# tusen-ai/SST

Hardware: AMD Instinct MI355X
Metric: LiDAR frames/sec (SST backbone fwd+bwd) at Waymo 0.32m voxels (higher is better)
Workload: dtype f32 (storage, accumulation, attention, LayerNorm, reductions: fp32; the dense products of the encoder layers from the EXACT three-way bf16 split of both fp32 operands, six bf16 MFMA products with fp32 accumulation - error vs float64 <= 2 x the fp32 matrix pipe's: tests/test_gpu_dense_f32x6.py)

## Files before the change

### include/sst_amd.h

```cpp
#ifndef SST_AMD_H
#define SST_AMD_H

#include <stdint.h>

#ifdef __cplusplus
extern "C" {
#endif

#define SST_OK 0
#define SST_ERR_ARG (-1)
#define SST_ERR_UNSUPPORTED (-2)
#define SST_ERR_KEYSPACE (-3)

typedef enum { SST_REDUCE_SUM = 0, SST_REDUCE_MEAN = 1, SST_REDUCE_MAX = 2 } sst_reduce_t;

const char* sst_version(void);

int sst_dynamic_voxelize_f32(const float* d_points, int64_t n, int64_t row_stride,
                             const float voxel_size[3], const float coors_range[6],
                             int32_t* d_coors, int64_t coors_stride, int coors_col0, int batch_idx,
                             void* stream);
void sst_dynamic_voxelize_grid(const float voxel_size[3], const float coors_range[6], int32_t grid_xyz[3]);

int64_t sst_scan_workspace_bytes(int64_t n);
// ... 184 lines not shown
int sst_add_layernorm_act_bwd_f32(const float* d_dy, const float* d_sum, const float* d_stats, const float* d_weight,
                                  const float* d_bias, int act, int64_t m, int c, float* d_dx, float* d_dweight,
                                  float* d_dbias, void* d_workspace, void* stream);
int sst_add_layernorm_fwd_f32(const float* d_x, const float* d_res, const float* d_weight, const float* d_bias,
                              int64_t m, int c, float eps, float* d_y, float* d_sum, float* d_stats,
                              void* stream);
int sst_add_layernorm_pos_fwd_f32(const float* d_x, const float* d_res, const float* d_weight, const float* d_bias, int64_t m,
                                  int c, float eps, float* d_y, float* d_sum, float* d_stats, const float* d_pos_table,
                                  const int32_t* d_pos_idx, float* d_y_plus_pos, void* stream);
int64_t sst_add_layernorm_bwd_workspace_bytes(int64_t m, int c);
int sst_add_layernorm_bwd_f32(const float* d_dy, const float* d_sum, const float* d_stats,
                              const float* d_weight, int64_t m, int c, float* d_dx, float* d_dweight,
                              float* d_dbias, void* d_workspace, void* stream);
int64_t sst_colsum_workspace_bytes(int64_t m, int c);
int sst_colsum_f32(const float* d_x, int64_t m, int c, int64_t ld, float* d_out, void* d_workspace, void* stream);

int64_t sst_weight_grad_workspace_bytes(int64_t m, int out, int in);
int sst_weight_grad_f32(const float* d_dy, const float* d_x, int64_t m, int out, int in, int64_t ld_dy,
                        int64_t ld_x, float* d_dw, float* d_db, void* d_workspace, void* stream);
typedef struct sst_wgrad_problem_f32 {
  const float* dy;
  const float* x;
  int64_t m, ld_dy, ld_x;
  float* dw;
  float* db;
  int32_t out, in;
  const float* x_add_rows;
  const int32_t* x_add_index;
} sst_wgrad_problem_f32;
int64_t sst_weight_grad_group_workspace_bytes(const sst_wgrad_problem_f32* problems, int n);
int sst_weight_grad_group_f32(const sst_wgrad_problem_f32* problems, int n, void* d_workspace, void* stream);
int64_t sst_weight_grad_group_f32x6_workspace_bytes(const sst_wgrad_problem_f32* problems, int n);
int sst_weight_grad_group_f32x6(const sst_wgrad_problem_f32* problems, int n, void* d_workspace, void* stream);

int64_t sst_bn_workspace_bytes(int64_t n, int c);
int sst_bn_stats_f32(const float* d_x, int64_t n, int c, int64_t ld, float* d_mean, float* d_var,
                     void* d_workspace, void* stream);
int sst_bn_act_fwd_f32(const float* d_x, int64_t n, int c, int64_t ldx, const float* d_scale,
                       const float* d_shift, int act, float* d_y, int64_t ldy, void* stream);
int sst_bn_act_bwd_reduce_f32(const float* d_dy, const float* d_x, int64_t n, int c, int64_t lddy, int64_t ldx,
                              const float* d_mean, const float* d_invstd, const float* d_scale,
                              const float* d_shift, int act, float* d_sum_g, float* d_sum_gxhat,
                              void* d_workspace, void* stream);
int sst_bn_act_bwd_apply_f32(const float* d_dy, const float* d_x, int64_t n, int c, int64_t lddy, int64_t ldx,
                             const float* d_mean, const float* d_invstd, const float* d_scale,
                             const float* d_shift, const float* d_coef_a, const float* d_coef_b, float coef_scale,
                             int act, float* d_dx, int64_t lddx, void* stream);
int sst_bn_prepare_f32(const float* d_x, int64_t n, int c, int64_t ld, const float* d_weight, const float* d_bias,
                       float eps, float* d_running_mean, float* d_running_var, float factor, float* d_out4,
                       void* d_workspace, void* stream);
int sst_bn_prepare_tracked_f32(const float* d_x, int64_t n, int c, int64_t ld, const float* d_weight,
                               const float* d_bias, float eps, float* d_running_mean, float* d_running_var,
                               float factor, int64_t* d_num_batches_tracked, float* d_out4, void* d_workspace,
                               void* stream);
int sst_vfe_linear_moments_f32(const float* d_x, int64_t ldx, int64_t n, int k, const float* d_w, int64_t ldw, int c,
                               float* d_y, int64_t ldy, void* d_workspace, void* stream);
int sst_bn_prepare_from_partials_f32(int64_t n, int c, const float* d_weight, const float* d_bias, float eps,
                                     float* d_running_mean, float* d_running_var, float factor,
                                     int64_t* d_num_batches_tracked, float* d_out4, void* d_workspace, void* stream);
int sst_bn_stats_from_partials_f32(int64_t n, int c, float* d_mean, float* d_var, void* d_workspace, void* stream);
int sst_bn_act_pool_bwd_reduce_f32(const float* d_dy, const float* d_x, int64_t n, int c, int64_t lddy, int64_t ldx,
                                   const float* d_mean, const float* d_invstd, const float* d_scale, const float* d_shift,
                                   int act, const int32_t* d_group, const int32_t* d_arg, const float* d_dpool, int64_t ldp,
                                   float* d_sum_g, float* d_sum_gxhat, void* d_workspace, void* stream);
int sst_bn_act_pool_bwd_apply_f32(const float* d_dy, const float* d_x, int64_t n, int c, int64_t lddy, int64_t ldx,
                                  const float* d_mean, const float* d_invstd, const float* d_scale, const float* d_shift,
// ... 352 lines not shown
```

### sst_amd/_lib.py

```python
import ctypes
import os
import subprocess

import torch

_HERE = os.path.dirname(os.path.abspath(__file__))
_CSRC = os.path.join(_HERE, 'csrc')
LIB_PATH = os.path.join(_CSRC, 'libsst_amd.so')

_lib = None

c_i64 = ctypes.c_int64
c_i32 = ctypes.c_int
c_f32 = ctypes.c_float
c_ptr = ctypes.c_void_p



class WgradProblemBF16(ctypes.Structure):
    _fields_ = [('a', c_ptr), ('b', c_ptr), ('lda', c_i64), ('ldb', c_i64), ('m', c_i64), ('out_w', c_ptr),
                ('out_b', c_ptr), ('p', ctypes.c_int32), ('bias_side', ctypes.c_int32),
                ('transpose_out', ctypes.c_int32), ('reserved', ctypes.c_int32)]


# ... 137 lines not shown
    'sst_sra_attn_fwd_ord_f32': (c_i32, [c_ptr, c_ptr, c_ptr, c_i64, c_i64, c_i64, c_ptr, c_ptr, c_ptr, c_i64, c_i32,
                                         c_f32, c_i32, c_i32, c_ptr, c_i64, c_ptr, c_ptr]),
    'sst_sra_attn_bwd_ord_f32': (c_i32, [c_ptr] * 6 + [c_i64] * 5 + [c_ptr, c_ptr, c_ptr, c_i64, c_i64, c_i32, c_f32,
                                                                     c_i32, c_i32, c_ptr, c_ptr, c_ptr,
                                                                     c_i64, c_i64, c_i64, c_ptr, c_ptr]),
    'sst_sra_attn_bwd_workspace_bytes': (c_i64, [c_i64, c_i32]),
    'sst_sra_attn_cos_fwd_f32': (c_i32, [c_ptr, c_ptr, c_ptr, c_i64, c_i64, c_i64, c_ptr, c_ptr, c_ptr, c_i64, c_i32,
                                         c_ptr, c_i32, c_ptr, c_i64, c_ptr, c_ptr]),
    'sst_sra_attn_cos_bwd_f32': (c_i32, [c_ptr] * 6 + [c_i64] * 5 + [c_ptr, c_ptr, c_ptr, c_i64, c_i64, c_i32, c_ptr,
                                                                     c_i32, c_ptr, c_ptr, c_ptr,
                                                                     c_i64, c_i64, c_i64, c_ptr, c_ptr]),
    'sst_sra_attn_fwd_bf16': (c_i32, [c_ptr, c_ptr, c_ptr, c_i64, c_i64, c_i64, c_ptr, c_ptr, c_i64, c_i32, c_f32, c_i32,
                                      c_ptr, c_i64, c_ptr, c_ptr]),
    'sst_sra_attn_bwd_bf16': (c_i32, [c_ptr] * 6 + [c_i64] * 5 + [c_ptr, c_ptr, c_i64, c_i32, c_f32, c_i32, c_ptr, c_ptr,
                                                                  c_ptr, c_i64, c_i64, c_i64, c_ptr]),
    'sst_sra_attn_bf16_profile_next': (c_i32, [c_i32, c_ptr, c_ptr]),
    'sst_sra_attn_fwd_ord_bf16': (c_i32, [c_ptr, c_ptr, c_ptr, c_i64, c_i64, c_i64, c_ptr, c_ptr, c_ptr, c_i64, c_i32, c_f32,
                                          c_i32, c_ptr, c_i64, c_ptr, c_ptr]),
    'sst_sra_attn_bwd_ord_bf16': (c_i32, [c_ptr] * 6 + [c_i64] * 5 + [c_ptr, c_ptr, c_ptr, c_i64, c_i32, c_f32, c_i32, c_ptr,
                                                                      c_ptr, c_ptr, c_i64, c_i64, c_i64, c_ptr]),
    'sst_sra_attn_cos_fwd_bf16': (c_i32, [c_ptr, c_ptr, c_ptr, c_i64, c_i64, c_i64, c_ptr, c_ptr, c_ptr, c_i64, c_i32, c_ptr,
                                          c_i32, c_ptr, c_i64, c_ptr, c_ptr]),
    'sst_sra_attn_cos_bwd_bf16': (c_i32, [c_ptr] * 6 + [c_i64] * 5 + [c_ptr, c_ptr, c_ptr, c_i64, c_i32, c_ptr, c_i32, c_ptr,
                                                                      c_ptr, c_ptr, c_i64, c_i64, c_i64, c_ptr, c_ptr]),
    'sst_add_layernorm_fwd_bf16': (c_i32, [c_ptr, c_ptr, c_ptr, c_ptr, c_i64, c_i32, c_f32, c_ptr, c_ptr, c_ptr, c_ptr,
                                           c_ptr, c_ptr, c_ptr]),
    'sst_add_layernorm_bwd_bf16': (c_i32, [c_ptr, c_ptr, c_ptr, c_ptr, c_ptr, c_i64, c_i32, c_ptr, c_ptr, c_ptr, c_ptr,
                                           c_ptr]),
    'sst_cast_add_pos_bf16': (c_i32, [c_ptr, c_i32, c_i64, c_i32, c_ptr, c_ptr, c_ptr, c_ptr]),
    'sst_weight_grad_group_workspace_bytes': (c_i64, [c_ptr, c_i32]),
    'sst_weight_grad_group_f32': (c_i32, [c_ptr, c_i32, c_ptr, c_ptr]),
    'sst_weight_grad_group_f32x6_workspace_bytes': (c_i64, [c_ptr, c_i32]),
    'sst_weight_grad_group_f32x6': (c_i32, [c_ptr, c_i32, c_ptr, c_ptr]),
    'sst_tall_linear_ln_f32': (c_i32, [c_ptr, c_i64, c_ptr, c_i64, c_ptr, c_i64, c_i32, c_ptr, c_i64, c_ptr, c_ptr, c_f32, c_ptr,
                                       c_ptr, c_ptr, c_ptr, c_ptr, c_ptr, c_ptr]),
    'sst_tall_linear_ln_f32x3': (c_i32, [c_ptr, c_i64, c_ptr, c_i64, c_ptr, c_i64, c_i32, c_ptr, c_i64, c_ptr, c_ptr, c_f32, c_ptr,
                                         c_ptr, c_ptr, c_ptr, c_ptr, c_ptr, c_ptr]),
    'sst_tall_linear_epi_f32x3': (c_i32, [c_ptr, c_i64, c_ptr, c_i64, c_i32, c_ptr, c_i64, c_i32, c_i32, c_i32, c_ptr, c_ptr,
                                          c_i64, c_ptr, c_i64, c_ptr]),
    'sst_tall_linear_ln_f32x6': (c_i32, [c_ptr, c_i64, c_ptr, c_i64, c_ptr, c_i64, c_i32, c_ptr, c_i64, c_ptr, c_ptr, c_f32, c_ptr,
                                         c_ptr, c_ptr, c_ptr, c_ptr, c_ptr, c_ptr]),
    'sst_tall_linear_epi_f32x6': (c_i32, [c_ptr, c_i64, c_ptr, c_i64, c_i32, c_ptr, c_i64, c_i32, c_i32, c_i32, c_ptr, c_ptr,
                                          c_i64, c_ptr, c_i64, c_ptr]),
    'sst_tall_linear_epi2_f32x6': (c_i32, [c_ptr, c_ptr, c_i32, c_i64, c_ptr, c_i64, c_i32, c_ptr, c_i64, c_i32, c_i32, c_i32,
                                           c_ptr, c_ptr, c_i64, c_ptr, c_i64, c_ptr]),
    'sst_add_layernorm_bwd2_f32': (c_i32, [c_ptr, c_ptr, c_ptr, c_ptr, c_ptr, c_i64, c_i32, c_ptr, c_ptr, c_ptr, c_ptr, c_ptr]),
    'sst_tall_linear_epi_f32': (c_i32, [c_ptr, c_i64, c_ptr, c_i64, c_i32, c_ptr, c_i64, c_i32, c_i32, c_i32, c_ptr, c_ptr,
                                        c_i64, c_ptr, c_i64, c_ptr]),
    'sst_tall_linear_bf16': (c_i32, [c_ptr, c_i64, c_ptr, c_ptr, c_i64, c_i32, c_i32, c_i32, c_ptr, c_ptr, c_i64, c_ptr,
                                     c_i64, c_ptr]),
    'sst_tall_linear_ln_bf16': (c_i32, [c_ptr, c_i64, c_ptr, c_ptr, c_i64, c_i32, c_ptr, c_i64, c_ptr, c_ptr, c_f32, c_ptr, c_ptr,
                                        c_ptr, c_ptr, c_ptr, c_ptr, c_ptr]),
    'sst_wgrad_group_workspace_bytes': (c_i64, [c_ptr, c_i32]),
    'sst_wgrad_group_bf16': (c_i32, [c_ptr, c_i32, c_ptr, c_ptr]),
    'sst_cast_group_bf16': (c_i32, [c_ptr, c_i32, c_ptr]),
    'sst_gather_rows_f32': (c_i32, [c_ptr, c_i64, c_ptr, c_i64, c_i32, c_f32, c_ptr, c_i64, c_ptr]),
    'sst_add_table_rows_f32': (c_i32, [c_ptr, c_i64, c_ptr, c_i64, c_ptr, c_i64, c_i32, c_ptr, c_i64, c_ptr]),
    'sst_scatter_rows_f32': (c_i32, [c_ptr, c_i64, c_ptr, c_i64, c_i32, c_ptr, c_i64, c_ptr]),
    'sst_add_layernorm_fwd_f32': (c_i32, [c_ptr, c_ptr, c_ptr, c_ptr, c_i64, c_i32, c_f32, c_ptr, c_ptr, c_ptr,
                                          c_ptr]),
    'sst_add_layernorm_bwd_workspace_bytes': (c_i64, [c_i64, c_i32]),
    'sst_add_layernorm_pos_fwd_f32': (c_i32, [c_ptr, c_ptr, c_ptr, c_ptr, c_i64, c_i32, c_f32, c_ptr, c_ptr, c_ptr, c_ptr, c_ptr,
                                              c_ptr, c_ptr]),
    'sst_add_layernorm_act_fwd_f32': (c_i32, [c_ptr, c_ptr, c_ptr, c_ptr, c_i64, c_i32, c_f32, c_i32, c_ptr, c_ptr, c_ptr,
                                              c_ptr]),
    'sst_add_layernorm_act_bwd_f32': (c_i32, [c_ptr, c_ptr, c_ptr, c_ptr, c_ptr, c_i32, c_i64, c_i32, c_ptr, c_ptr, c_ptr,
# ... 241 lines not shown
```

### sst_amd/csrc/wgrad_x6.hip

```cpp
#include <math.h>
#include <stdlib.h>
#include "common.h"

namespace {

typedef float f32x4 __attribute__((ext_vector_type(4)));
typedef float f32x2 __attribute__((ext_vector_type(2)));
typedef unsigned u32x4 __attribute__((ext_vector_type(4)));
typedef unsigned u32x2 __attribute__((ext_vector_type(2)));
typedef __bf16 bf16x8 __attribute__((ext_vector_type(8)));
typedef __bf16 bf16x2 __attribute__((ext_vector_type(2)));

__device__ __forceinline__ unsigned pack2(float lo, float hi) {
  const f32x2 v = {lo, hi};
  return __builtin_bit_cast(unsigned, __builtin_convertvector(v, bf16x2));
}
__device__ __forceinline__ float lo_f(unsigned p) { return __uint_as_float(p << 16); }
__device__ __forceinline__ float hi_f(unsigned p) { return __uint_as_float(p & 0xffff0000u); }
__device__ __forceinline__ f32x4 mma32(u32x4 a, u32x4 b, f32x4 c) {
  return __builtin_amdgcn_mfma_f32_16x16x32_bf16(__builtin_bit_cast(bf16x8, a), __builtin_bit_cast(bf16x8, b), c, 0, 0, 0);
}
__device__ __forceinline__ void split2(float a, float b, unsigned& p0, unsigned& p1, unsigned& p2) {
  p0 = pack2(a, b);
  const float ra = a - lo_f(p0), rb = b - hi_f(p0);
  p1 = pack2(ra, rb);
  p2 = pack2(ra - lo_f(p1), rb - hi_f(p1));
}

constexpr int kMaxProblems = 8;
constexpr int kTile = 128;
constexpr int kStep = 32;
constexpr int kTileLds = 1040;
constexpr int kImage = 8 * kTileLds;
constexpr int kStage = 2 * 3 * kImage;
constexpr int kLdsBytes = 2 * kStage;

struct x6_problem {
  const float* dy;
  const float* x;
  int64_t m, ld_dy, ld_x;
  int out, in;
  int tile0;
  int db_off;
  float* dw;
  float* db;
  const float* x_add_rows;
  const int32_t* x_add_index;
};
struct x6_group {
  x6_problem p[kMaxProblems];
  int n, tiles, slices;
  int64_t tokens_per_slice;
};

__global__ __launch_bounds__(512, 2) void wgrad_x6_k(const x6_group G, float* __restrict__ part, float* __restrict__ dbp) {
  extern __shared__ __attribute__((aligned(16))) unsigned char lds[];
  const int tid = threadIdx.x, lane = tid & 63, wave = tid >> 6;
  const int l15 = lane & 15, g = lane >> 4;
  const int tile = blockIdx.x / G.slices, slice = blockIdx.x - tile * G.slices;
  int pi = 0;
#pragma unroll
  for (int q = 1; q < kMaxProblems; ++q)
    if (q < G.n && tile >= G.p[q].tile0) pi = q;
  const x6_problem P = G.p[pi];
  const int tiles_k = P.in / kTile;
  const int tl = tile - P.tile0, tn = tl / tiles_k, tk = tl - tn * tiles_k;
  const int n0 = tn * kTile, k0 = tk * kTile;
  const int64_t t_begin = (int64_t)slice * G.tokens_per_slice;
  int64_t t_end = t_begin + G.tokens_per_slice;
  t_end = t_end < P.m ? t_end : P.m;

  const int op = tid >> 8, tq = (tid >> 5) & 7, cg = tid & 31;
  const float* src = op == 0 ? P.dy + n0 + 4 * cg : P.x + k0 + 4 * cg;
  const int64_t ld = op == 0 ? P.ld_dy : P.ld_x;
  const int st_off = (cg >> 2) * kTileLds + (tq & 1) * 512 + (tq >> 1) * 128 + (cg & 3) * 32;
  constexpr int kPf = 2;
  f32x4 rows[kPf][4];
  const int64_t t_last = t_end > 0 ? t_end - 1 : 0;
  const bool xadd = op == 1 && P.x_add_rows != nullptr;
  const float* addsrc = xadd ? P.x_add_rows + k0 + 4 * cg : nullptr;
  f32x4 prow[kPf][4];
  int32_t pidx[4] = {0, 0, 0, 0};
  auto load_idx = [&](int64_t t0) {
#pragma unroll
    for (int r = 0; r < 4; ++r) {
      int64_t t = t0 + 4 * tq + r;
      t = t < t_last ? t : t_last;
      pidx[r] = P.x_add_index[t];
    }
  };
  auto load_rows = [&](int64_t t0, f32x4 (&dst)[4], f32x4 (&pdst)[4]) {
#pragma unroll
    for (int r = 0; r < 4; ++r) {
      int64_t t = t0 + 4 * tq + r;
      t = t < t_last ? t : t_last;
      dst[r] = *(const f32x4*)(src + t * ld);
    }
    if (xadd) {
#pragma unroll
      for (int r = 0; r < 4; ++r) pdst[r] = *(const f32x4*)(addsrc + (int64_t)pidx[r] * P.in);
      load_idx(t0 + kStep);
    }
  };
  float bsum[4] = {0.f, 0.f, 0.f, 0.f};
  u32x4 img[3][2];
  auto split_col = [&](int e, int64_t t0, const f32x4 (&rws)[4], const f32x4 (&prw)[4]) {
    float v[4];
#pragma unroll
    for (int r = 0; r < 4; ++r) v[r] = (t0 + 4 * tq + r < t_end) ? (xadd ? rws[r][e] + prw[r][e] : rws[r][e]) : 0.f;
    if (op == 0) bsum[e] += (v[0] + v[1]) + (v[2] + v[3]);
    unsigned a0, a1, a2, b0, b1, b2;
    split2(v[0], v[1], a0, a1, a2);
    split2(v[2], v[3], b0, b1, b2);
    img[0][e >> 1][2 * (e & 1)] = a0;
    img[0][e >> 1][2 * (e & 1) + 1] = b0;
    img[1][e >> 1][2 * (e & 1)] = a1;
    img[1][e >> 1][2 * (e & 1) + 1] = b1;
    img[2][e >> 1][2 * (e & 1)] = a2;
    img[2][e >> 1][2 * (e & 1) + 1] = b2;
  };
  auto store_img = [&](int buf) {
    unsigned char* base = lds + buf * kStage + op * 3 * kImage + st_off;
#pragma unroll
    for (int im = 0; im < 3; ++im) {
      *(u32x4*)(base + im * kImage) = img[im][0];
      *(u32x4*)(base + im * kImage + 16) = img[im][1];
    }
  };
  const int wn = wave & 3, wk = wave >> 2;
  const int frag_off = g * 128 + l15 * 8;
  f32x4 acc[4][2], acl[4][2];
#pragma unroll
  for (int a = 0; a < 4; ++a)
#pragma unroll
    for (int b = 0; b < 2; ++b) acc[a][b] = acl[a][b] = (f32x4){0.f, 0.f, 0.f, 0.f};
  auto frag = [&](const unsigned char* image, int tile16) -> u32x4 {
    const unsigned char* p = image + tile16 * kTileLds + frag_off;
    const u32x2 lo = *(const u32x2*)p, hi = *(const u32x2*)(p + 512);
    return (u32x4){lo[0], lo[1], hi[0], hi[1]};
  };

  if (xadd) load_idx(t_begin);
#pragma unroll
  for (int u = 0; u < kPf; ++u) load_rows(t_begin + (int64_t)u * kStep, rows[u], prow[u]);
#pragma unroll
  for (int e = 0; e < 4; ++e) split_col(e, t_begin, rows[0], prow[0]);
  store_img(0);
  load_rows(t_begin + (int64_t)kPf * kStep, rows[0], prow[0]);
  __syncthreads();
  const int64_t n_steps = (t_end - t_begin + kStep - 1) / kStep;
  for (int64_t s0 = 0; s0 < n_steps; s0 += kPf) {
#pragma unroll
    for (int u = 0; u < kPf; ++u) {
      const int64_t s = s0 + u;
      if (s >= n_steps) break;
      const int64_t t1 = t_begin + (s + 1) * kStep;
      const unsigned char* dyi = lds + (u & 1) * kStage;
      const unsigned char* xi = dyi + 3 * kImage;
      u32x4 b0[2], b1[2], b2[2];
#pragma unroll
      for (int b = 0; b < 2; ++b) {
        b0[b] = frag(dyi, 2 * wn + b);
        b1[b] = frag(dyi + kImage, 2 * wn + b);
        b2[b] = frag(dyi + 2 * kImage, 2 * wn + b);
      }
#pragma unroll
      for (int a = 0; a < 4; ++a) {
        const u32x4 a0 = frag(xi, 4 * wk + a), a1 = frag(xi + kImage, 4 * wk + a), a2 = frag(xi + 2 * kImage, 4 * wk + a);
#pragma unroll
        for (int b = 0; b < 2; ++b) acl[a][b] = mma32(a2, b0[b], acl[a][b]);
#pragma unroll
        for (int b = 0; b < 2; ++b) acl[a][b] = mma32(a0, b2[b], acl[a][b]);
#pragma unroll
        for (int b = 0; b < 2; ++b) acl[a][b] = mma32(a1, b1[b], acl[a][b]);
#pragma unroll
        for (int b = 0; b < 2; ++b) acl[a][b] = mma32(a1, b0[b], acl[a][b]);
#pragma unroll
        for (int b = 0; b < 2; ++b) acl[a][b] = mma32(a0, b1[b], acl[a][b]);
#pragma unroll
        for (int b = 0; b < 2; ++b) acc[a][b] = mma32(a0, b0[b], acc[a][b]);
        split_col(a, t1, rows[(u + 1) % kPf], prow[(u + 1) % kPf]);
      }
      store_img((u + 1) & 1);
      load_rows(t1 + (int64_t)kPf * kStep, rows[(u + 1) % kPf], prow[(u + 1) % kPf]);
      __syncthreads();
    }
  }
#pragma unroll
  for (int a = 0; a < 4; ++a)
#pragma unroll
    for (int b = 0; b < 2; ++b) acc[a][b] += acl[a][b];
  float* dst = part + ((int64_t)tile * G.slices + slice) * (kTile * kTile);
#pragma unroll
  for (int a = 0; a < 4; ++a)
#pragma unroll
    for (int b = 0; b < 2; ++b)
      *(f32x4*)(dst + (32 * wn + 16 * b + l15) * kTile + 64 * wk + 16 * a + 4 * g) = acc[a][b];
  if (P.db_off >= 0 && tk == 0) {
    float* red = (float*)lds;
    if (op == 0) *(f32x4*)(red + tq * 128 + 4 * cg) = (f32x4){bsum[0], bsum[1], bsum[2], bsum[3]};
    __syncthreads();
    if (tid < 128) {
      float s = 0.f;
#pragma unroll
      for (int q = 0; q < 8; ++q) s += red[q * 128 + tid];
      dbp[((int64_t)P.db_off + n0 + tid) * G.slices + slice] = s;
    }
  }
}

struct x6_riders {
  sst_colsum_rider r[2];
  int n, blocks0;
};

constexpr int kRedQuads = 32, kRedGroups = 8;

__global__ __launch_bounds__(256) void wgrad_x6_reduce_k(const x6_group G, const float* __restrict__ part,
                                                         const float* __restrict__ dbp, int rider_blocks,
                                                         const x6_riders R) {
  __shared__ double red[kRedGroups][kRedQuads][4];
  if ((int)blockIdx.x < rider_blocks) {
    const int second = (int)blockIdx.x >= R.blocks0 ? 1 : 0;
    const sst_colsum_rider& J = R.r[second];
    const int rblk = (int)blockIdx.x - (second ? R.blocks0 : 0);
    float* fr = (float*)&red[0][0][0];
    const int cx = threadIdx.x & 31, gq = threadIdx.x >> 5;
    const int i = rblk * 32 + cx;
    float acc[4] = {0.f, 0.f, 0.f, 0.f};
    if (i < J.width) {
      const float* src = J.partials + i;
      for (int base = 0; base < J.nb; base += 512) {
        float v[16][4];
#pragma unroll
        for (int it = 0; it < 16; ++it)
#pragma unroll
          for (int j = 0; j < 4; ++j) {
            const int b = base + 32 * it + gq + 8 * j;
            v[it][j] = src[(int64_t)(b < J.nb ? b : J.nb - 1) * J.width];
          }
#pragma unroll
        for (int it = 0; it < 16; ++it)
#pragma unroll
          for (int j = 0; j < 4; ++j)
            if (base + 32 * it + gq + 8 * j < J.nb) acc[j] += v[it][j];
      }
    }
#pragma unroll
    for (int j = 0; j < 4; ++j) fr[(gq + 8 * j) * 33 + cx] = acc[j];
    __syncthreads();
    if (gq == 0 && i < J.width) {
      float t = 0.f;
#pragma unroll
      for (int k = 0; k < 32; ++k) t += fr[k * 33 + cx];
      if (i < J.split)
        J.out0[i] = t;
      else
        J.out1[i - J.split] = t;
    }
    return;
  }
  const int blk = (int)blockIdx.x - rider_blocks;
  const int ql = threadIdx.x & (kRedQuads - 1), sg = threadIdx.x / kRedQuads;
  const int64_t quad = (int64_t)blk * kRedQuads + ql;
  const int64_t tile = quad / (kTile * kTile / 4);
  const int e4 = (int)(quad - tile * (kTile * kTile / 4));
  double d0 = 0.0, d1 = 0.0, d2 = 0.0, d3 = 0.0;
  if (tile < G.tiles) {
    const float* src = part + tile * G.slices * (int64_t)(kTile * kTile) + 4 * e4;
#pragma unroll 8
    for (int q = sg; q < G.slices; q += kRedGroups) {
      const f32x4 v = *(const f32x4*)(src + (int64_t)q * (kTile * kTile));
      d0 += v[0], d1 += v[1], d2 += v[2], d3 += v[3];
    }
  }
  red[sg][ql][0] = d0, red[sg][ql][1] = d1, red[sg][ql][2] = d2, red[sg][ql][3] = d3;
  __syncthreads();
  if (sg == 0 && tile < G.tiles) {
    f32x4 s;
#pragma unroll
    for (int r = 0; r < 4; ++r) {
      double t = 0.0;
#pragma unroll
      for (int k = 0; k < kRedGroups; ++k) t += red[k][ql][r];
      s[r] = (float)t;
    }
    int pi = 0;
#pragma unroll
    for (int q = 1; q < kMaxProblems; ++q)
      if (q < G.n && tile >= G.p[q].tile0) pi = q;
    const int tiles_k = G.p[pi].in / kTile;
    const int tl = (int)tile - G.p[pi].tile0, tn = tl / tiles_k, tk = tl - tn * tiles_k;
    const int n = tn * kTile + e4 / 32, k = tk * kTile + (e4 % 32) * 4;
    *(f32x4*)(G.p[pi].dw + (int64_t)n * G.p[pi].in + k) = s;
  }
  const int64_t col = (int64_t)blk * 256 + threadIdx.x;
  int base = 0;
  for (int q = 0; q < G.n; ++q) {
    if (G.p[q].db_off < 0) continue;
    if (col >= base && col < base + G.p[q].out) {
      const float* src = dbp + ((int64_t)G.p[q].db_off + (col - base)) * G.slices;
      double s = 0.0;
      for (int i = 0; i < G.slices; ++i) s += src[i];
      G.p[q].db[col - base] = (float)s;
    }
    base += G.p[q].out;
  }
}

bool aligned16(const void* p) { return ((uintptr_t)p & 15) == 0; }

struct x6_plan {
  x6_group g;
  int64_t part_bytes, db_bytes;
};

bool make_plan(const sst_wgrad_problem_f32* pr, int n, x6_plan* plan) {
  if (!pr || n < 1 || n > kMaxProblems) return false;
  x6_group& G = plan->g;
  G.n = n;
  int tiles = 0, db_cols = 0;
  int64_t m = pr[0].m;
  for (int i = 0; i < n; ++i) {
    const sst_wgrad_problem_f32& p = pr[i];
    if (p.m != m || p.m < 1 || p.out < kTile || p.in < kTile || (p.out % kTile) || (p.in % kTile) || (p.ld_dy & 3) ||
        (p.ld_x & 3) || !p.dy || !p.x || !p.dw || !aligned16(p.dy) || !aligned16(p.x) || !aligned16(p.dw))
      return false;
    G.p[i].dy = p.dy;
    G.p[i].x = p.x;
    G.p[i].m = p.m;
    G.p[i].ld_dy = p.ld_dy;
    G.p[i].ld_x = p.ld_x;
    G.p[i].out = p.out;
    G.p[i].in = p.in;
    G.p[i].tile0 = tiles;
    G.p[i].db_off = p.db ? db_cols : -1;
    G.p[i].dw = p.dw;
    G.p[i].db = p.db;
    if ((p.x_add_rows != nullptr) != (p.x_add_index != nullptr) || (p.x_add_rows && !aligned16(p.x_add_rows))) return false;
    G.p[i].x_add_rows = p.x_add_rows;
    G.p[i].x_add_index = p.x_add_index;
    tiles += (p.out / kTile) * (p.in / kTile);
    if (p.db) db_cols += p.out;
  }
  G.tiles = tiles;
  int slices = (256 / tiles) & ~7;
  if (slices < 8) slices = 8;
  const int64_t max_slices = sst_div_up(m, (int64_t)kStep);
  while (slices > 8 && slices > max_slices) slices -= 8;
  G.slices = slices;
  G.tokens_per_slice = sst_align_up(sst_div_up(m, (int64_t)slices), (int64_t)kStep);
  plan->part_bytes = sst_align_up((int64_t)tiles * slices * kTile * kTile * 4, 256);
  plan->db_bytes = sst_align_up((int64_t)(db_cols > 0 ? db_cols : 1) * slices * 4, 256);
  return true;
}

}

extern "C" {

int64_t sst_weight_grad_group_f32x6_workspace_bytes(const sst_wgrad_problem_f32* problems, int n) {
  x6_plan plan;
  if (!make_plan(problems, n, &plan)) return SST_ERR_UNSUPPORTED;
  return plan.part_bytes + plan.db_bytes;
}

}

int sst_internal_weight_grad_group_f32x6(const sst_wgrad_problem_f32* problems, int n, void* d_workspace,
                                         const sst_colsum_rider* riders, int n_riders, void* stream) {
  x6_plan plan;
  if (!make_plan(problems, n, &plan)) return SST_ERR_UNSUPPORTED;
  if (!d_workspace || !aligned16(d_workspace)) return SST_ERR_ARG;
  hipStream_t st = (hipStream_t)stream;
  float* part = (float*)d_workspace;
  float* dbp = (float*)((char*)d_workspace + plan.part_bytes);
  static unsigned long long configured = 0;
  if (sst_first_use_on_device(&configured)) {
    SST_HIP(hipFuncSetAttribute((const void*)wgrad_x6_k, hipFuncAttributeMaxDynamicSharedMemorySize, kLdsBytes));
    sst_mark_device(&configured);
  }
  const int64_t quads = (int64_t)plan.g.tiles * (kTile * kTile / 4);
  const int tile_blocks = (int)sst_div_up(quads, (int64_t)kRedQuads);
  if (n_riders < 0 || n_riders > 2 || (n_riders > 0 && !riders)) return SST_ERR_ARG;
  x6_riders R;
  R.n = n_riders, R.blocks0 = 0;
  int extra = 0;
  for (int i = 0; i < n_riders; ++i) {
    const sst_colsum_rider& q = riders[i];
    if (!q.partials || q.nb < 1 || q.width < 1 || !q.out0 || !q.out1) return SST_ERR_ARG;
    R.r[i] = q;
    if (i == 0) R.blocks0 = (q.width + 31) / 32;
    extra += (q.width + 31) / 32;
  }
  hipLaunchKernelGGL(wgrad_x6_k, dim3((unsigned)(plan.g.tiles * plan.g.slices)), dim3(512), kLdsBytes, st, plan.g, part, dbp);
  hipLaunchKernelGGL(wgrad_x6_reduce_k, dim3((unsigned)(tile_blocks + extra)), dim3(256), 0, st, plan.g, part, dbp, extra, R);
  SST_LAUNCH_CHECK();
  return SST_OK;
}

extern "C" {

int sst_weight_grad_group_f32x6(const sst_wgrad_problem_f32* problems, int n, void* d_workspace, void* stream) {
  return sst_internal_weight_grad_group_f32x6(problems, n, d_workspace, nullptr, 0, stream);
}

}
```

Measured before the change: 97.91.

## Pair adjacent weight-grad tiles per block to reuse the shared operand split

The f32x6 weight-gradient kernel now processes units of two adjacent 128x128 output tiles along the in or out dimension. Each unit loads and splits the shared operand (dy or x) once and reuses it for both tiles. It uses 256-thread blocks with a three-block LDS stage and larger per-wave accumulators. Leftover odd tiles run as single-tile units. The host planner picks separate slice counts for pairs and singles from a cost model over 256 CUs. The reduce kernel and bias reduction are updated for the new partial layout, and a partition query API is added. This cuts redundant global loads and bf16 splitting, at the cost of more register pressure, occupancy 1, and fewer blocks per tile.

```diff
diff --git a/include/sst_amd.h b/include/sst_amd.h
--- a/include/sst_amd.h
+++ b/include/sst_amd.h
@@ -240,6 +240,9 @@
 int sst_weight_grad_group_f32(const sst_wgrad_problem_f32* problems, int n, void* d_workspace, void* stream);
 int64_t sst_weight_grad_group_f32x6_workspace_bytes(const sst_wgrad_problem_f32* problems, int n);
 int sst_weight_grad_group_f32x6(const sst_wgrad_problem_f32* problems, int n, void* d_workspace, void* stream);
+int sst_weight_grad_group_f32x6_partition(const sst_wgrad_problem_f32* problems, int n, int max_units, int* n_units,
+                                          int32_t* unit_problem, int32_t* unit_tiles, int32_t* unit_slices,
+                                          int64_t* unit_tokens_per_slice);
 
 int64_t sst_bn_workspace_bytes(int64_t n, int c);
 int sst_bn_stats_f32(const float* d_x, int64_t n, int c, int64_t ld, float* d_mean, float* d_var,
diff --git a/sst_amd/_lib.py b/sst_amd/_lib.py
--- a/sst_amd/_lib.py
+++ b/sst_amd/_lib.py
@@ -193,6 +193,7 @@
     'sst_weight_grad_group_f32': (c_i32, [c_ptr, c_i32, c_ptr, c_ptr]),
     'sst_weight_grad_group_f32x6_workspace_bytes': (c_i64, [c_ptr, c_i32]),
     'sst_weight_grad_group_f32x6': (c_i32, [c_ptr, c_i32, c_ptr, c_ptr]),
+    'sst_weight_grad_group_f32x6_partition': (c_i32, [c_ptr, c_i32, c_i32, c_ptr, c_ptr, c_ptr, c_ptr, c_ptr]),
     'sst_tall_linear_ln_f32': (c_i32, [c_ptr, c_i64, c_ptr, c_i64, c_ptr, c_i64, c_i32, c_ptr, c_i64, c_ptr, c_ptr, c_f32, c_ptr,
                                        c_ptr, c_ptr, c_ptr, c_ptr, c_ptr, c_ptr]),
     'sst_tall_linear_ln_f32x3': (c_i32, [c_ptr, c_i64, c_ptr, c_i64, c_ptr, c_i64, c_i32, c_ptr, c_i64, c_ptr, c_ptr, c_f32, c_ptr,
diff --git a/sst_amd/csrc/wgrad_x6.hip b/sst_amd/csrc/wgrad_x6.hip
--- a/sst_amd/csrc/wgrad_x6.hip
+++ b/sst_amd/csrc/wgrad_x6.hip
@@ -29,18 +29,27 @@
 
 constexpr int kMaxProblems = 8;
 constexpr int kTile = 128;
+constexpr int kTile2 = kTile * kTile;
 constexpr int kStep = 32;
 constexpr int kTileLds = 1040;
 constexpr int kImage = 8 * kTileLds;
-constexpr int kStage = 2 * 3 * kImage;
+constexpr int kBlock = 3 * kImage;
+constexpr int kStage = 3 * kBlock;
 constexpr int kLdsBytes = 2 * kStage;
+constexpr int kThreads = 256;
+constexpr int kCus = 256;
+constexpr double kSingleCost = 0.58;
+
+enum { kDirNone = 0, kDirIn = 1, kDirOut = 2 };
 
 struct x6_problem {
   const float* dy;
   const float* x;
   int64_t m, ld_dy, ld_x;
   int out, in;
-  int tile0;
+  int dir;
+  int ppl;
+  int pair0, sing0;
   int db_off;
   float* dw;
   float* db;
@@ -49,164 +58,251 @@
 };
 struct x6_group {
   x6_problem p[kMaxProblems];
-  int n, tiles, slices;
-  int64_t tokens_per_slice;
+  int n, pairs, singles;
+  int slices_pair, slices_single;
+  int db_stride;
+  int64_t tps_pair, tps_single;
 };
-
-__global__ __launch_bounds__(512, 2) void wgrad_x6_k(const x6_group G, float* __restrict__ part, float* __restrict__ dbp) {
-  extern __shared__ __attribute__((aligned(16))) unsigned char lds[];
+struct x6_unit {
+  int pi, tn, tk;
+};
+
+__host__ __device__ __forceinline__ x6_unit locate(const x6_group& G, bool pair, int u) {
+  int pi = 0;
+#pragma unroll
+  for (int q = 1; q < kMaxProblems; ++q)
+    if (q < G.n && u >= (pair ? G.p[q].pair0 : G.p[q].sing0)) pi = q;
+  const x6_problem& P = G.p[pi];
+  const int tiles_n = P.out / kTile, tiles_k = P.in / kTile;
+  x6_unit r;
+  r.pi = pi;
+  if (pair) {
+    const int ul = u - P.pair0, line = ul / P.ppl, j = ul - line * P.ppl;
+    if (P.dir == kDirIn)
+      r.tn = line, r.tk = 2 * j;
+    else
+      r.tk = line, r.tn = 2 * j;
+  } else {
+    const int ul = u - P.sing0;
+    if (P.dir == kDirNone)
+      r.tn = ul / tiles_k, r.tk = ul - r.tn * tiles_k;
+    else if (P.dir == kDirIn)
+      r.tn = ul, r.tk = tiles_k - 1;
+    else
+      r.tk = ul, r.tn = tiles_n - 1;
+  }
+  return r;
+}
+
+template <int NDY, int NX>
+__device__ __forceinline__ void unit_body(const x6_problem& P, unsigned char* lds, const int n0, const int k0,
+                                          const int64_t t_begin, const int64_t t_end, float* __restrict__ dst,
+                                          float* __restrict__ dbp_col, const int db_stride, const bool write_db) {
+  constexpr int NBK = NDY + NX;
+  constexpr int NS = NBK == 3 ? 8 : 4;
+  constexpr bool kStreamX = NX == 1;
+  constexpr bool kXadd = NX == 1;
   const int tid = threadIdx.x, lane = tid & 63, wave = tid >> 6;
   const int l15 = lane & 15, g = lane >> 4;
-  const int tile = blockIdx.x / G.slices, slice = blockIdx.x - tile * G.slices;
-  int pi = 0;
-#pragma unroll
-  for (int q = 1; q < kMaxProblems; ++q)
-    if (q < G.n && tile >= G.p[q].tile0) pi = q;
-  const x6_problem P = G.p[pi];
-  const int tiles_k = P.in / kTile;
-  const int tl = tile - P.tile0, tn = tl / tiles_k, tk = tl - tn * tiles_k;
-  const int n0 = tn * kTile, k0 = tk * kTile;
-  const int64_t t_begin = (int64_t)slice * G.tokens_per_slice;
-  int64_t t_end = t_begin + G.tokens_per_slice;
-  t_end = t_end < P.m ? t_end : P.m;
-
-  const int op = tid >> 8, tq = (tid >> 5) & 7, cg = tid & 31;
-  const float* src = op == 0 ? P.dy + n0 + 4 * cg : P.x + k0 + 4 * cg;
-  const int64_t ld = op == 0 ? P.ld_dy : P.ld_x;
+
+  const int tq = tid >> 5, cg = tid & 31;
+  const char* src[NBK];
+  int ldb[NBK];
+#pragma unroll
+  for (int b = 0; b < NDY; ++b) src[b] = (const char*)(P.dy + t_begin * P.ld_dy + n0 + kTile * b + 4 * cg), ldb[b] = (int)(4 * P.ld_dy);
+#pragma unroll
+  for (int b = 0; b < NX; ++b) src[NDY + b] = (const char*)(P.x + t_begin * P.ld_x + k0 + kTile * b + 4 * cg), ldb[NDY + b] = (int)(4 * P.ld_x);
   const int st_off = (cg >> 2) * kTileLds + (tq & 1) * 512 + (tq >> 1) * 128 + (cg & 3) * 32;
-  constexpr int kPf = 2;
-  f32x4 rows[kPf][4];
-  const int64_t t_last = t_end > 0 ? t_end - 1 : 0;
-  const bool xadd = op == 1 && P.x_add_rows != nullptr;
+  f32x4 rows[NBK][4];
+  const int rel_last = (int)(t_end - 1 - t_begin);
+  const int rel0 = 4 * tq;
+  const bool xadd = kXadd && P.x_add_rows != nullptr;
   const float* addsrc = xadd ? P.x_add_rows + k0 + 4 * cg : nullptr;
-  f32x4 prow[kPf][4];
+  f32x4 prow[4];
   int32_t pidx[4] = {0, 0, 0, 0};
-  auto load_idx = [&](int64_t t0) {
+  const int32_t* idxsrc = xadd ? P.x_add_index + t_begin : nullptr;
+  auto load_idx = [&](int step) {
 #pragma unroll
     for (int r = 0; r < 4; ++r) {
-      int64_t t = t0 + 4 * tq + r;
-      t = t < t_last ? t : t_last;
-      pidx[r] = P.x_add_index[t];
+      const int rel = step * kStep + rel0 + r;
+      pidx[r] = idxsrc[rel < rel_last ? rel : rel_last];
     }
   };
-  auto load_rows = [&](int64_t t0, f32x4 (&dst)[4], f32x4 (&pdst)[4]) {
+  auto load_block = [&](int b, int step) {
 #pragma unroll
     for (int r = 0; r < 4; ++r) {
-      int64_t t = t0 + 4 * tq + r;
-      t = t < t_last ? t : t_last;
-      dst[r] = *(const f32x4*)(src + t * ld);
-    }
-    if (xadd) {
-#pragma unroll
-      for (int r = 0; r < 4; ++r) pdst[r] = *(const f32x4*)(addsrc + (int64_t)pidx[r] * P.in);
-      load_idx(t0 + kStep);
+      const int rel = step * kStep + rel0 + r;
+      rows[b][r] = *(const f32x4*)(src[b] + (int64_t)(rel < rel_last ? rel : rel_last) * ldb[b]);
+    }
+    if (kXadd && b == NBK - 1 && xadd) {
+#pragma unroll
+      for (int r = 0; r < 4; ++r) prow[r] = *(const f32x4*)(addsrc + (int64_t)pidx[r] * P.in);
+      load_idx(step + 1);
     }
   };
-  float bsum[4] = {0.f, 0.f, 0.f, 0.f};
-  u32x4 img[3][2];
-  auto split_col = [&](int e, int64_t t0, const f32x4 (&rws)[4], const f32x4 (&prw)[4]) {
+  float bsum[NDY][4];
+#pragma unroll
+  for (int b = 0; b < NDY; ++b)
+#pragma unroll
+    for (int e = 0; e < 4; ++e) bsum[b][e] = 0.f;
+  u32x4 img[3];
+  auto split_col = [&](int b, int e, int rem) {
     float v[4];
 #pragma unroll
-    for (int r = 0; r < 4; ++r) v[r] = (t0 + 4 * tq + r < t_end) ? (xadd ? rws[r][e] + prw[r][e] : rws[r][e]) : 0.f;
-    if (op == 0) bsum[e] += (v[0] + v[1]) + (v[2] + v[3]);
+    for (int r = 0; r < 4; ++r) {
+      const float val = (kXadd && b == NBK - 1 && xadd) ? rows[b][r][e] + prow[r][e] : rows[b][r][e];
+      v[r] = (4 * tq + r < rem) ? val : 0.f;
+    }
+    if (b < NDY) bsum[b < NDY ? b : 0][e] += (v[0] + v[1]) + (v[2] + v[3]);
     unsigned a0, a1, a2, b0, b1, b2;
     split2(v[0], v[1], a0, a1, a2);
     split2(v[2], v[3], b0, b1, b2);
-    img[0][e >> 1][2 * (e & 1)] = a0;
-    img[0][e >> 1][2 * (e & 1) + 1] = b0;
-    img[1][e >> 1][2 * (e & 1)] = a1;
-    img[1][e >> 1][2 * (e & 1) + 1] = b1;
-    img[2][e >> 1][2 * (e & 1)] = a2;
-    img[2][e >> 1][2 * (e & 1) + 1] = b2;
+    img[0][2 * (e & 1)] = a0;
+    img[0][2 * (e & 1) + 1] = b0;
+    img[1][2 * (e & 1)] = a1;
+    img[1][2 * (e & 1) + 1] = b1;
+    img[2][2 * (e & 1)] = a2;
+    img[2][2 * (e & 1) + 1] = b2;
   };
-  auto store_img = [&](int buf) {
-    unsigned char* base = lds + buf * kStage + op * 3 * kImage + st_off;
-#pragma unroll
-    for (int im = 0; im < 3; ++im) {
-      *(u32x4*)(base + im * kImage) = img[im][0];
-      *(u32x4*)(base + im * kImage + 16) = img[im][1];
-    }
+  auto store_img = [&](int b, int half, int buf) {
+    unsigned char* base = lds + buf * kStage + b * kBlock + st_off + 16 * half;
+#pragma unroll
+    for (int im = 0; im < 3; ++im) *(u32x4*)(base + im * kImage) = img[im];
   };
-  const int wn = wave & 3, wk = wave >> 2;
+  const int n_steps = t_end > t_begin ? (int)((t_end - t_begin + kStep - 1) / kStep) : 0;
+  auto step_rem = [&](int step) -> int {
+    const int d = rel_last + 1 - step * kStep;
+    return d < 0 ? 0 : (d > kStep ? kStep : d);
+  };
+  const int wl = wave & 1, wh = wave >> 1;
   const int frag_off = g * 128 + l15 * 8;
-  f32x4 acc[4][2], acl[4][2];
-#pragma unroll
-  for (int a = 0; a < 4; ++a)
-#pragma unroll
-    for (int b = 0; b < 2; ++b) acc[a][b] = acl[a][b] = (f32x4){0.f, 0.f, 0.f, 0.f};
-  auto frag = [&](const unsigned char* image, int tile16) -> u32x4 {
-    const unsigned char* p = image + tile16 * kTileLds + frag_off;
+  const int held_off = (NDY == 2 ? wh : NX == 2 ? 1 + wh : 0) * kBlock + 4 * wl * kTileLds + frag_off;
+  const int str_off = (NDY == 2 ? 2 : NX == 2 ? 0 : 1) * kBlock + (NBK == 2 ? 4 * wh * kTileLds : 0) + frag_off;
+  f32x4 acc[NS][4], acl[NS][4];
+#pragma unroll
+  for (int s = 0; s < NS; ++s)
+#pragma unroll
+    for (int h = 0; h < 4; ++h) acc[s][h] = acl[s][h] = (f32x4){0.f, 0.f, 0.f, 0.f};
+  auto frag = [&](const unsigned char* p) -> u32x4 {
     const u32x2 lo = *(const u32x2*)p, hi = *(const u32x2*)(p + 512);
     return (u32x4){lo[0], lo[1], hi[0], hi[1]};
   };
 
-  if (xadd) load_idx(t_begin);
-#pragma unroll
-  for (int u = 0; u < kPf; ++u) load_rows(t_begin + (int64_t)u * kStep, rows[u], prow[u]);
-#pragma unroll
-  for (int e = 0; e < 4; ++e) split_col(e, t_begin, rows[0], prow[0]);
-  store_img(0);
-  load_rows(t_begin + (int64_t)kPf * kStep, rows[0], prow[0]);
+  if (xadd) load_idx(0);
+  {
+    const int rem0 = step_rem(0);
+#pragma unroll
+    for (int b = 0; b < NBK; ++b) load_block(b, 0);
+#pragma unroll
+    for (int b = 0; b < NBK; ++b) {
+#pragma unroll
+      for (int e = 0; e < 4; ++e) {
+        split_col(b, e, rem0);
+        if (e & 1) store_img(b, e >> 1, 0);
+      }
+      load_block(b, 1);
+    }
+  }
   __syncthreads();
-  const int64_t n_steps = (t_end - t_begin + kStep - 1) / kStep;
-  for (int64_t s0 = 0; s0 < n_steps; s0 += kPf) {
-#pragma unroll
-    for (int u = 0; u < kPf; ++u) {
-      const int64_t s = s0 + u;
-      if (s >= n_steps) break;
-      const int64_t t1 = t_begin + (s + 1) * kStep;
-      const unsigned char* dyi = lds + (u & 1) * kStage;
-      const unsigned char* xi = dyi + 3 * kImage;
-      u32x4 b0[2], b1[2], b2[2];
-#pragma unroll
-      for (int b = 0; b < 2; ++b) {
-        b0[b] = frag(dyi, 2 * wn + b);
-        b1[b] = frag(dyi + kImage, 2 * wn + b);
-        b2[b] = frag(dyi + 2 * kImage, 2 * wn + b);
+  for (int s0 = 0; s0 < n_steps; s0 += 2) {
+#pragma unroll
+    for (int u = 0; u < 2; ++u) {
+      if (s0 + u >= n_steps) break;
+      const int rem1 = step_rem(s0 + u + 1);
+      const unsigned char* held = lds + u * kStage + held_off;
+      const unsigned char* strm = lds + u * kStage + str_off;
+      u32x4 hf[4][3], sf[3];
+#pragma unroll
+      for (int h = 0; h < 4; ++h)
+#pragma unroll
+        for (int i = 0; i < 3; ++i) hf[h][i] = frag(held + i * kImage + h * kTileLds);
+#pragma unroll
+      for (int i = 0; i < 3; ++i) sf[i] = frag(strm + i * kImage);
+#pragma unroll
+      for (int s = 0; s < NS; ++s) {
+        u32x4 nf[3];
+        if (s + 1 < NS) {
+#pragma unroll
+          for (int i = 0; i < 3; ++i) nf[i] = frag(strm + i * kImage + (s + 1) * kTileLds);
+        }
+        auto prod = [&](int i, int j, f32x4 (&c)[4]) {
+#pragma unroll
+          for (int h = 0; h < 4; ++h) c[h] = kStreamX ? mma32(sf[i], hf[h][j], c[h]) : mma32(hf[h][i], sf[j], c[h]);
+        };
+        prod(2, 0, acl[s]);
+        prod(0, 2, acl[s]);
+        prod(1, 1, acl[s]);
+        prod(1, 0, acl[s]);
+        prod(0, 1, acl[s]);
+        prod(0, 0, acc[s]);
+#pragma unroll
+        for (int j = s * (4 * NBK) / NS; j < (s + 1) * (4 * NBK) / NS; ++j) {
+          split_col(j >> 2, j & 3, rem1);
+          if (j & 1) store_img(j >> 2, (j & 3) >> 1, u ^ 1);
+          if ((j & 3) == 3) load_block(j >> 2, s0 + u + 2);
+        }
+        if (s + 1 < NS) {
+#pragma unroll
+          for (int i = 0; i < 3; ++i) sf[i] = nf[i];
+        }
       }
-#pragma unroll
-      for (int a = 0; a < 4; ++a) {
-        const u32x4 a0 = frag(xi, 4 * wk + a), a1 = frag(xi + kImage, 4 * wk + a), a2 = frag(xi + 2 * kImage, 4 * wk + a);
-#pragma unroll
-        for (int b = 0; b < 2; ++b) acl[a][b] = mma32(a2, b0[b], acl[a][b]);
-#pragma unroll
-        for (int b = 0; b < 2; ++b) acl[a][b] = mma32(a0, b2[b], acl[a][b]);
-#pragma unroll
-        for (int b = 0; b < 2; ++b) acl[a][b] = mma32(a1, b1[b], acl[a][b]);
-#pragma unroll
-        for (int b = 0; b < 2; ++b) acl[a][b] = mma32(a1, b0[b], acl[a][b]);
-#pragma unroll
-        for (int b = 0; b < 2; ++b) acl[a][b] = mma32(a0, b1[b], acl[a][b]);
-#pragma unroll
-        for (int b = 0; b < 2; ++b) acc[a][b] = mma32(a0, b0[b], acc[a][b]);
-        split_col(a, t1, rows[(u + 1) % kPf], prow[(u + 1) % kPf]);
+      __syncthreads();
+    }
+  }
+#pragma unroll
+  for (int s = 0; s < NS; ++s)
+#pragma unroll
+    for (int h = 0; h < 4; ++h) {
+      const f32x4 v = acc[s][h] + acl[s][h];
+      int row, col, half = 0;
+      if (NDY == 2)
+        half = wh, row = 64 * wl + 16 * h + l15, col = 16 * s + 4 * g;
+      else if (NX == 2)
+        half = wh, row = 16 * s + l15, col = 64 * wl + 16 * h + 4 * g;
+      else
+        row = 64 * wl + 16 * h + l15, col = 64 * wh + 16 * s + 4 * g;
+      *(f32x4*)(dst + half * kTile2 + row * kTile + col) = v;
+    }
+  if (write_db) {
+    float* red = (float*)lds;
+#pragma unroll
+    for (int b = 0; b < NDY; ++b) *(f32x4*)(red + (b * 8 + tq) * kTile + 4 * cg) = (f32x4){bsum[b][0], bsum[b][1], bsum[b][2], bsum[b][3]};
+    __syncthreads();
+    if (tid < kTile) {
+#pragma unroll
+      for (int b = 0; b < NDY; ++b) {
+        float s = 0.f;
+#pragma unroll
+        for (int q = 0; q < 8; ++q) s += red[(b * 8 + q) * kTile + tid];
+        dbp_col[(int64_t)(kTile * b + tid) * db_stride] = s;
       }
-      store_img((u + 1) & 1);
-      load_rows(t1 + (int64_t)kPf * kStep, rows[(u + 1) % kPf], prow[(u + 1) % kPf]);
-      __syncthreads();
-    }
-  }
-#pragma unroll
-  for (int a = 0; a < 4; ++a)
-#pragma unroll
-    for (int b = 0; b < 2; ++b) acc[a][b] += acl[a][b];
-  float* dst = part + ((int64_t)tile * G.slices + slice) * (kTile * kTile);
-#pragma unroll
-  for (int a = 0; a < 4; ++a)
-#pragma unroll
-    for (int b = 0; b < 2; ++b)
-      *(f32x4*)(dst + (32 * wn + 16 * b + l15) * kTile + 64 * wk + 16 * a + 4 * g) = acc[a][b];
-  if (P.db_off >= 0 && tk == 0) {
-    float* red = (float*)lds;
-    if (op == 0) *(f32x4*)(red + tq * 128 + 4 * cg) = (f32x4){bsum[0], bsum[1], bsum[2], bsum[3]};
-    __syncthreads();
-    if (tid < 128) {
-      float s = 0.f;
-#pragma unroll
-      for (int q = 0; q < 8; ++q) s += red[q * 128 + tid];
-      dbp[((int64_t)P.db_off + n0 + tid) * G.slices + slice] = s;
-    }
-  }
+    }
+  }
+}
+
+__global__ __launch_bounds__(kThreads, 1) void wgrad_x6_k(const x6_group G, float* __restrict__ part, float* __restrict__ dbp) {
+  extern __shared__ __attribute__((aligned(16))) unsigned char lds[];
+  const int pair_blocks = G.pairs * G.slices_pair;
+  const bool pair = (int)blockIdx.x < pair_blocks;
+  const int id = pair ? (int)blockIdx.x : (int)blockIdx.x - pair_blocks;
+  const int S = pair ? G.slices_pair : G.slices_single;
+  const int64_t tps = pair ? G.tps_pair : G.tps_single;
+  const int u = id / S, slice = id - u * S;
+  const x6_unit U = locate(G, pair, u);
+  const x6_problem& P = G.p[U.pi];
+  const int n0 = U.tn * kTile, k0 = U.tk * kTile;
+  const int64_t t_begin = (int64_t)slice * tps;
+  int64_t t_end = t_begin + tps;
+  t_end = t_end < P.m ? t_end : P.m;
+  float* dst = pair ? part + (int64_t)id * (2 * kTile2) : part + (int64_t)pair_blocks * (2 * kTile2) + (int64_t)id * kTile2;
+  const bool write_db = P.db_off >= 0 && U.tk == 0;
+  float* dbp_col = dbp + ((int64_t)(P.db_off >= 0 ? P.db_off : 0) + n0) * G.db_stride + slice;
+  if (!pair)
+    unit_body<1, 1>(P, lds, n0, k0, t_begin, t_end, dst, dbp_col, G.db_stride, write_db);
+  else if (P.dir == kDirOut)
+    unit_body<2, 1>(P, lds, n0, k0, t_begin, t_end, dst, dbp_col, G.db_stride, write_db);
+  else
+    unit_body<1, 2>(P, lds, n0, k0, t_begin, t_end, dst, dbp_col, G.db_stride, write_db);
 }
 
 struct x6_riders {
@@ -263,20 +359,26 @@
   const int blk = (int)blockIdx.x - rider_blocks;
   const int ql = threadIdx.x & (kRedQuads - 1), sg = threadIdx.x / kRedQuads;
   const int64_t quad = (int64_t)blk * kRedQuads + ql;
-  const int64_t tile = quad / (kTile * kTile / 4);
-  const int e4 = (int)(quad - tile * (kTile * kTile / 4));
+  const int tile = (int)(quad / (kTile2 / 4));
+  const int e4 = (int)(quad - (int64_t)tile * (kTile2 / 4));
+  const int n_tiles = 2 * G.pairs + G.singles;
+  const bool pair = tile < 2 * G.pairs;
+  const int u = pair ? tile >> 1 : tile - 2 * G.pairs, half = pair ? tile & 1 : 0;
+  const int S = pair ? G.slices_pair : G.slices_single;
   double d0 = 0.0, d1 = 0.0, d2 = 0.0, d3 = 0.0;
-  if (tile < G.tiles) {
-    const float* src = part + tile * G.slices * (int64_t)(kTile * kTile) + 4 * e4;
+  if (tile < n_tiles) {
+    const int64_t stride = pair ? 2 * kTile2 : kTile2;
+    const float* src = part + (pair ? ((int64_t)u * S * 2 + half) * kTile2
+                                    : (int64_t)G.pairs * G.slices_pair * (2 * kTile2) + (int64_t)u * S * kTile2) + 4 * e4;
 #pragma unroll 8
-    for (int q = sg; q < G.slices; q += kRedGroups) {
-      const f32x4 v = *(const f32x4*)(src + (int64_t)q * (kTile * kTile));
+    for (int q = sg; q < S; q += kRedGroups) {
+      const f32x4 v = *(const f32x4*)(src + (int64_t)q * stride);
       d0 += v[0], d1 += v[1], d2 += v[2], d3 += v[3];
     }
   }
   red[sg][ql][0] = d0, red[sg][ql][1] = d1, red[sg][ql][2] = d2, red[sg][ql][3] = d3;
   __syncthreads();
-  if (sg == 0 && tile < G.tiles) {
+  if (sg == 0 && tile < n_tiles) {
     f32x4 s;
 #pragma unroll
     for (int r = 0; r < 4; ++r) {
@@ -285,24 +387,24 @@
       for (int k = 0; k < kRedGroups; ++k) t += red[k][ql][r];
       s[r] = (float)t;
     }
-    int pi = 0;
-#pragma unroll
-    for (int q = 1; q < kMaxProblems; ++q)
-      if (q < G.n && tile >= G.p[q].tile0) pi = q;
-    const int tiles_k = G.p[pi].in / kTile;
-    const int tl = (int)tile - G.p[pi].tile0, tn = tl / tiles_k, tk = tl - tn * tiles_k;
+    const x6_unit U = locate(G, pair, u);
+    const x6_problem& P = G.p[U.pi];
+    const int tn = U.tn + (pair && P.dir == kDirOut ? half : 0), tk = U.tk + (pair && P.dir == kDirIn ? half : 0);
     const int n = tn * kTile + e4 / 32, k = tk * kTile + (e4 % 32) * 4;
-    *(f32x4*)(G.p[pi].dw + (int64_t)n * G.p[pi].in + k) = s;
+    *(f32x4*)(P.dw + (int64_t)n * P.in + k) = s;
   }
   const int64_t col = (int64_t)blk * 256 + threadIdx.x;
   int base = 0;
   for (int q = 0; q < G.n; ++q) {
     if (G.p[q].db_off < 0) continue;
     if (col >= base && col < base + G.p[q].out) {
-      const float* src = dbp + ((int64_t)G.p[q].db_off + (col - base)) * G.slices;
+      const int c = (int)(col - base);
+      const bool in_pair = G.p[q].dir == kDirIn || (G.p[q].dir == kDirOut && c / kTile < 2 * G.p[q].ppl);
+      const int Sb = in_pair ? G.slices_pair : G.slices_single;
+      const float* src = dbp + ((int64_t)G.p[q].db_off + c) * G.db_stride;
       double s = 0.0;
-      for (int i = 0; i < G.slices; ++i) s += src[i];
-      G.p[q].db[col - base] = (float)s;
+      for (int i = 0; i < Sb; ++i) s += src[i];
+      G.p[q].db[c] = (float)s;
     }
     base += G.p[q].out;
   }
@@ -319,7 +421,7 @@
   if (!pr || n < 1 || n > kMaxProblems) return false;
   x6_group& G = plan->g;
   G.n = n;
-  int tiles = 0, db_cols = 0;
+  int pairs = 0, singles = 0, db_cols = 0;
   int64_t m = pr[0].m;
   for (int i = 0; i < n; ++i) {
     const sst_wgrad_problem_f32& p = pr[i];
@@ -333,25 +435,47 @@
     G.p[i].ld_x = p.ld_x;
     G.p[i].out = p.out;
     G.p[i].in = p.in;
-    G.p[i].tile0 = tiles;
     G.p[i].db_off = p.db ? db_cols : -1;
     G.p[i].dw = p.dw;
     G.p[i].db = p.db;
     if ((p.x_add_rows != nullptr) != (p.x_add_index != nullptr) || (p.x_add_rows && !aligned16(p.x_add_rows))) return false;
     G.p[i].x_add_rows = p.x_add_rows;
     G.p[i].x_add_index = p.x_add_index;
-    tiles += (p.out / kTile) * (p.in / kTile);
+    const int tiles_n = p.out / kTile, tiles_k = p.in / kTile;
+    const bool two_x_ok = p.x_add_rows == nullptr;
+    int dir = kDirNone, len = 1, lines = tiles_n * tiles_k;
+    if (tiles_k % 2 == 0 && two_x_ok)
+      dir = kDirIn, len = tiles_k, lines = tiles_n;
+    else if (tiles_n >= 2)
+      dir = kDirOut, len = tiles_n, lines = tiles_k;
+    else if (tiles_k >= 2 && two_x_ok)
+      dir = kDirIn, len = tiles_k, lines = tiles_n;
+    G.p[i].dir = dir;
+    G.p[i].ppl = len / 2;
+    G.p[i].pair0 = pairs;
+    G.p[i].sing0 = singles;
+    pairs += lines * (len / 2);
+    singles += lines * (len & 1);
     if (p.db) db_cols += p.out;
   }
-  G.tiles = tiles;
-  int slices = (256 / tiles) & ~7;
-  if (slices < 8) slices = 8;
+  G.pairs = pairs, G.singles = singles;
+  int sp = 8, ss = 8;
+  double best = 0.0;
+  for (int a = 8; a <= kCus; a += 8)
+    for (int b = 8; b <= kCus; b += 8) {
+      if (pairs * a + singles * b > kCus) break;
+      const double cp = pairs ? 1.0 / a : 0.0, cs = singles ? kSingleCost / b : 0.0, c = cp > cs ? cp : cs;
+      if (best == 0.0 || c < best) best = c, sp = pairs ? a : 8, ss = singles ? b : 8;
+    }
   const int64_t max_slices = sst_div_up(m, (int64_t)kStep);
-  while (slices > 8 && slices > max_slices) slices -= 8;
-  G.slices = slices;
-  G.tokens_per_slice = sst_align_up(sst_div_up(m, (int64_t)slices), (int64_t)kStep);
-  plan->part_bytes = sst_align_up((int64_t)tiles * slices * kTile * kTile * 4, 256);
-  plan->db_bytes = sst_align_up((int64_t)(db_cols > 0 ? db_cols : 1) * slices * 4, 256);
+  while (sp > 8 && sp > max_slices) sp -= 8;
+  while (ss > 8 && ss > max_slices) ss -= 8;
+  G.slices_pair = sp, G.slices_single = ss;
+  G.db_stride = sp > ss ? sp : ss;
+  G.tps_pair = sst_align_up(sst_div_up(m, (int64_t)sp), (int64_t)kStep);
+  G.tps_single = sst_align_up(sst_div_up(m, (int64_t)ss), (int64_t)kStep);
+  plan->part_bytes = sst_align_up(((int64_t)pairs * sp * 2 + (int64_t)singles * ss) * kTile2 * 4, 256);
+  plan->db_bytes = sst_align_up((int64_t)(db_cols > 0 ? db_cols : 1) * G.db_stride * 4, 256);
   return true;
 }
 
@@ -380,8 +504,8 @@
     SST_HIP(hipFuncSetAttribute((const void*)wgrad_x6_k, hipFuncAttributeMaxDynamicSharedMemorySize, kLdsBytes));
     sst_mark_device(&configured);
   }
-  const int64_t quads = (int64_t)plan.g.tiles * (kTile * kTile / 4);
-  const int tile_blocks = (int)sst_div_up(quads, (int64_t)kRedQuads);
+  const int tile_blocks = (2 * plan.g.pairs + plan.g.singles) * (kTile2 / 4 / kRedQuads);
+  const int unit_blocks = plan.g.pairs * plan.g.slices_pair + plan.g.singles * plan.g.slices_single;
   if (n_riders < 0 || n_riders > 2 || (n_riders > 0 && !riders)) return SST_ERR_ARG;
   x6_riders R;
   R.n = n_riders, R.blocks0 = 0;
@@ -393,7 +517,7 @@
     if (i == 0) R.blocks0 = (q.width + 31) / 32;
     extra += (q.width + 31) / 32;
   }
-  hipLaunchKernelGGL(wgrad_x6_k, dim3((unsigned)(plan.g.tiles * plan.g.slices)), dim3(512), kLdsBytes, st, plan.g, part, dbp);
+  hipLaunchKernelGGL(wgrad_x6_k, dim3((unsigned)unit_blocks), dim3(kThreads), kLdsBytes, st, plan.g, part, dbp);
   hipLaunchKernelGGL(wgrad_x6_reduce_k, dim3((unsigned)(tile_blocks + extra)), dim3(256), 0, st, plan.g, part, dbp, extra, R);
   SST_LAUNCH_CHECK();
   return SST_OK;
@@ -405,4 +529,27 @@
   return sst_internal_weight_grad_group_f32x6(problems, n, d_workspace, nullptr, 0, stream);
 }
 
-}
+int sst_weight_grad_group_f32x6_partition(const sst_wgrad_problem_f32* problems, int n, int max_units, int* n_units,
+                                          int32_t* unit_problem, int32_t* unit_tiles, int32_t* unit_slices,
+                                          int64_t* unit_tokens_per_slice) {
+  x6_plan plan;
+  if (!make_plan(problems, n, &plan)) return SST_ERR_UNSUPPORTED;
+  const x6_group& G = plan.g;
+  if (!n_units) return SST_ERR_ARG;
+  *n_units = G.pairs + G.singles;
+  if (max_units < *n_units || !unit_problem || !unit_tiles || !unit_slices || !unit_tokens_per_slice) return SST_ERR_ARG;
+  for (int i = 0; i < G.pairs + G.singles; ++i) {
+    const bool pair = i < G.pairs;
+    const x6_unit U = locate(G, pair, pair ? i : i - G.pairs);
+    const x6_problem& P = G.p[U.pi];
+    const int tiles_k = P.in / kTile;
+    unit_problem[i] = U.pi;
+    unit_tiles[2 * i] = U.tn * tiles_k + U.tk;
+    unit_tiles[2 * i + 1] = !pair ? -1 : P.dir == kDirIn ? U.tn * tiles_k + U.tk + 1 : (U.tn + 1) * tiles_k + U.tk;
+    unit_slices[i] = pair ? G.slices_pair : G.slices_single;
+    unit_tokens_per_slice[i] = pair ? G.tps_pair : G.tps_single;
+  }
+  return SST_OK;
+}
+
+}
```

Result: no change. 98.88, median of 2 (+1.0%).
